# Megvii-CSG/MegReader

Hardware: AMD Instinct MI355X
Metric: training images/sec, CRNN-CTC 32x128 crops, batch 256 per GPU (higher is better)
Workload: dtype bf16; 1 GPU; CRNN + 1D-CTC training step (BASELINE.json configs[1]): 32x128 crops, T=33, C=38, Adam; global_batch=256, per_gpu_batch=256, parallelism=dp1, launch=hipGraph replay

## Files before the change

megreader_amd/csrc/stem.hip:

```cpp
#include "common.h"
#include "../../include/megreader_hip.h"

namespace mr {

constexpr int STEM_COUT = 64;
constexpr int STEM_BWD_GROUPS = 1024;

template <typename T> __device__ __forceinline__ float round_as(float v) { return to_f32(from_f32<T>(v)); }

template <typename T, int CIN>
__device__ __forceinline__ void stem_stage_patch(float* patch, const float* __restrict__ x, int n, int ph, int H,
                                                 int W) {
  const int PW = W + 2;
  for (int r = 0; r < 4; ++r) {
    const int row = 2 * ph - 1 + r;
    const bool rv = row >= 0 && row < H;
    for (int j = threadIdx.x; j < CIN * W; j += blockDim.x) {
      const int c = j / W, col = j - c * W;
      const float v = rv ? x[((long long)(n * CIN + c) * H + row) * W + col] : 0.f;
      patch[(r * PW + col + 1) * CIN + c] = round_as<T>(v);
    }
  }
  if (threadIdx.x < 4 * 2 * CIN) {
    const int r = threadIdx.x / (2 * CIN), rem = threadIdx.x - r * 2 * CIN;
    const int side = rem / CIN, c = rem - side * CIN;
    patch[(r * PW + (side ? W + 1 : 0)) * CIN + c] = 0.f;
  }
}

template <typename T, int CIN>
__global__ __launch_bounds__(256) void stem_fwd_kernel(const float* __restrict__ x, const float* __restrict__ w,
                                                       long long wsk, long long wsc, long long wsr, long long wss,
                                                       const float* __restrict__ bias, T* __restrict__ y,
                                                       unsigned char* __restrict__ code, int N, int H, int W) {
  extern __shared__ float patch[];
  constexpr int KT = 9 * CIN;
  const int lane = threadIdx.x & 63, wv = threadIdx.x >> 6, nwv = blockDim.x >> 6;
  const int Ho = H / 2, Wo = W / 2, PW = W + 2;
  float wr[KT];
#pragma unroll
  for (int dr = 0; dr < 3; ++dr)
#pragma unroll
    for (int ds = 0; ds < 3; ++ds)
#pragma unroll
      for (int c = 0; c < CIN; ++c)
        wr[(dr * 3 + ds) * CIN + c] = round_as<T>(w[lane * wsk + c * wsc + dr * wsr + ds * wss]);
  const float b = bias ? bias[lane] : 0.f;
  const int per = (Wo + nwv - 1) / nwv;
  for (int strip = blockIdx.x; strip < N * Ho; strip += gridDim.x) {
    const int n = strip / Ho, ph = strip - n * Ho;
    __syncthreads();
    stem_stage_patch<T, CIN>(patch, x, n, ph, H, W);
    __syncthreads();
    const int pw1 = min(Wo, (wv + 1) * per);
    for (int pw = wv * per; pw < pw1; ++pw) {
      float P[4][4 * CIN];
#pragma unroll
      for (int r = 0; r < 4; ++r)
#pragma unroll
        for (int i = 0; i < 4 * CIN; ++i) P[r][i] = patch[(r * PW + 2 * pw) * CIN + i];
      float best = 0.f;
      int q = 0;
#pragma unroll
      for (int qq = 0; qq < 4; ++qq) {
        const int a = qq >> 1, bq = qq & 1;
        float acc = b;
#pragma unroll
        for (int dr = 0; dr < 3; ++dr)
#pragma unroll
          for (int i = 0; i < 3 * CIN; ++i) acc = fmaf(wr[dr * 3 * CIN + i], P[a + dr][bq * CIN + i], acc);
        if (qq == 0 || acc > best) {
          best = acc;
          q = qq;
        }
      }
      const bool pos = best > 0.f;
      const long long o = ((long long)strip * Wo + pw) * STEM_COUT + lane;
      y[o] = from_f32<T>(pos ? best : 0.f);
      code[o] = (unsigned char)(q | (pos ? 4 : 0));
    }
  }
}

template <typename T, int CIN>
__global__ __launch_bounds__(256) void stem_bwd_kernel(const T* __restrict__ dy, const unsigned char* __restrict__ code,
                                                       const float* __restrict__ x, float* __restrict__ partial, int N,
                                                       int H, int W) {
  extern __shared__ float patch[];
  constexpr int KT = 9 * CIN;
  __shared__ float red[4][KT + 1][STEM_COUT];
  const int lane = threadIdx.x & 63, wv = threadIdx.x >> 6, nwv = blockDim.x >> 6;
  const int Ho = H / 2, Wo = W / 2, PW = W + 2;
  float acc[KT];
#pragma unroll
  for (int k = 0; k < KT; ++k) acc[k] = 0.f;
  float accb = 0.f;
  const int per = (Wo + nwv - 1) / nwv;
  for (int strip = blockIdx.x; strip < N * Ho; strip += gridDim.x) {
    const int n = strip / Ho, ph = strip - n * Ho;
    __syncthreads();
    stem_stage_patch<T, CIN>(patch, x, n, ph, H, W);
    __syncthreads();
    const int pw1 = min(Wo, (wv + 1) * per);
    for (int pw = wv * per; pw < pw1; ++pw) {
      const long long o = ((long long)strip * Wo + pw) * STEM_COUT + lane;
      const int cd = code[o];
      const float g = (cd & 4) ? to_f32(dy[o]) : 0.f;
      const int q = cd & 3;
      float P[4][4 * CIN];
#pragma unroll
      for (int r = 0; r < 4; ++r)
#pragma unroll
        for (int i = 0; i < 4 * CIN; ++i) P[r][i] = patch[(r * PW + 2 * pw) * CIN + i];
      accb += g;
#pragma unroll
      for (int qq = 0; qq < 4; ++qq) {
        const int a = qq >> 1, bq = qq & 1;
        const float gq = (q == qq) ? g : 0.f;
#pragma unroll
        for (int dr = 0; dr < 3; ++dr)
#pragma unroll
          for (int i = 0; i < 3 * CIN; ++i)
            acc[dr * 3 * CIN + i] = fmaf(gq, P[a + dr][bq * CIN + i], acc[dr * 3 * CIN + i]);
      }
    }
  }
  __syncthreads();
#pragma unroll
  for (int k = 0; k < KT; ++k) red[wv][k][lane] = acc[k];
  red[wv][KT][lane] = accb;
  __syncthreads();
  for (int i = threadIdx.x; i < (KT + 1) * STEM_COUT; i += blockDim.x) {
    const int k = i / STEM_COUT, o = i - k * STEM_COUT;
    float s = 0.f;
    for (int v = 0; v < nwv; ++v) s += red[v][k][o];
    partial[(long long)blockIdx.x * (KT + 1) * STEM_COUT + i] = s;
  }
}

template <int CIN>
__device__ __forceinline__ void stem_stage_patch_bf16(bf16_t* patch, const float* __restrict__ x, int n, int ph,
                                                      int H, int W) {
  const int PW = W + 2;
  const int wv = threadIdx.x >> 6, lane = threadIdx.x & 63;
  const int rbase = (wv & 1) * 2;
  for (int col = lane + 64 * (wv >> 1); col < W; col += 128) {
    float v[2][CIN];
#pragma unroll
    for (int rr = 0; rr < 2; ++rr) {
      const int row = 2 * ph - 1 + rbase + rr;
      const bool rv = row >= 0 && row < H;
#pragma unroll
      for (int c = 0; c < CIN; ++c) v[rr][c] = rv ? x[((long long)(n * CIN + c) * H + row) * W + col] : 0.f;
    }
#pragma unroll
    for (int rr = 0; rr < 2; ++rr)
#pragma unroll
      for (int c = 0; c < CIN; ++c) patch[((rbase + rr) * PW + col + 1) * CIN + c] = (bf16_t)v[rr][c];
  }
  if (threadIdx.x < 4 * 2 * CIN) {
    const int r = threadIdx.x / (2 * CIN), rem = threadIdx.x - r * 2 * CIN;
    const int side = rem / CIN, c = rem - side * CIN;
    patch[(r * PW + (side ? W + 1 : 0)) * CIN + c] = (bf16_t)0.f;
  }
}

template <int CIN>
__global__ void stem_pack_kernel(const float* __restrict__ w, long long wsk, long long wsc, long long wsr,
                                 long long wss, bf16_t* __restrict__ wpack) {
  constexpr int KT = 9 * CIN;
  for (int i = threadIdx.x; i < STEM_COUT * 32; i += blockDim.x) {
    const int ch = i >> 5, k = i & 31;
    const int dr = k / (3 * CIN), rem = k - dr * 3 * CIN, ds = rem / CIN, c = rem - ds * CIN;
    wpack[i] = (bf16_t)(k < KT ? w[ch * wsk + c * wsc + dr * wsr + ds * wss] : 0.f);
  }
}

template <int CIN>
__global__ __launch_bounds__(256, 3) void stem_fwd_mfma_kernel(const float* __restrict__ x,
                                                            const bf16_t* __restrict__ wpack,
                                                            const float* __restrict__ bias, bf16_t* __restrict__ y,
                                                            unsigned char* __restrict__ code, int N, int H, int W) {
  extern __shared__ float patch_raw[];
  bf16_t* patch = (bf16_t*)patch_raw;
  constexpr int KT = 9 * CIN;
  const int lane = threadIdx.x & 63, wv = threadIdx.x >> 6, l15 = lane & 15, lg = lane >> 4;
  const int Ho = H / 2, Wo = W / 2, PW = W + 2, ROW = PW * CIN;
  bf16x8 wf[4];
#pragma unroll
  for (int ct = 0; ct < 4; ++ct) {
    const int ch = (l15 >> 2) * 16 + ct * 4 + (l15 & 3);
    wf[ct] = *(const bf16x8*)(wpack + ch * 32 + 8 * lg);
  }
  f32x4 bv[4];
#pragma unroll
  for (int ct = 0; ct < 4; ++ct)
    bv[ct] = bias ? *(const f32x4*)(bias + lg * 16 + ct * 4) : f32x4{0.f, 0.f, 0.f, 0.f};
  int koff[8];
#pragma unroll
  for (int i = 0; i < 8; ++i) {
    const int k = 8 * lg + i;
    const int dr = k / (3 * CIN), rem = k - dr * 3 * CIN;
    koff[i] = k < KT ? dr * ROW + rem : 0;
  }

  for (int strip = blockIdx.x; strip < N * Ho; strip += gridDim.x) {
    const int n = strip / Ho, ph = strip - n * Ho;
    __syncthreads();
    stem_stage_patch_bf16<CIN>(patch, x, n, ph, H, W);
    __syncthreads();
    for (int pw0 = wv * 16; pw0 < Wo; pw0 += 64) {
      const int pw = pw0 + l15;
      bf16x8 xf[4];
#pragma unroll
      for (int qq = 0; qq < 4; ++qq) {
        const int base = ((qq >> 1) * PW + 2 * pw + (qq & 1)) * CIN;
#pragma unroll
        for (int i = 0; i < 8; ++i) xf[qq][i] = patch[base + koff[i]];
      }
      bf16_t yo[16];
      unsigned char co[16];
#pragma unroll
      for (int ct = 0; ct < 4; ++ct) {
        f32x4 acc[4];
#pragma unroll
        for (int qq = 0; qq < 4; ++qq)
          acc[qq] = __builtin_amdgcn_mfma_f32_16x16x32_bf16(wf[ct], xf[qq], f32x4{0.f, 0.f, 0.f, 0.f}, 0, 0, 0);
#pragma unroll
        for (int r = 0; r < 4; ++r) {
          const float a0 = acc[0][r], a1 = acc[1][r], a2 = acc[2][r], a3 = acc[3][r];
          const bool c1 = a1 > a0, c2 = a3 > a2;
          const float m01 = c1 ? a1 : a0, m23 = c2 ? a3 : a2;
          const bool c3 = m23 > m01;
          const int q = c3 ? (c2 ? 3 : 2) : (c1 ? 1 : 0);
          const float best = (c3 ? m23 : m01) + bv[ct][r];
          const bool pos = best > 0.f;
          yo[ct * 4 + r] = (bf16_t)(pos ? best : 0.f);
          co[ct * 4 + r] = (unsigned char)(pos ? (q | 4) : q);
        }
      }
      const long long o = ((long long)strip * Wo + pw) * STEM_COUT + lg * 16;
      *(uint4*)(y + o) = *(const uint4*)&yo[0];
      *(uint4*)(y + o + 8) = *(const uint4*)&yo[8];
      *(uint4*)(code + o) = *(const uint4*)&co[0];
    }
  }
}

template <int CIN>
__global__ __launch_bounds__(256, 4) void stem_bwd_mfma_kernel(const bf16_t* __restrict__ dy,
                                                            const unsigned char* __restrict__ code,
                                                            const float* __restrict__ x, float* __restrict__ partial,
                                                            int N, int H, int W) {
  extern __shared__ float patch_raw[];
  bf16_t* patch = (bf16_t*)patch_raw;
  const unsigned short* patch16 = (const unsigned short*)patch_raw;
  const unsigned short* dy16 = (const unsigned short*)dy;
  constexpr int KT = 9 * CIN;
  __shared__ float red[4][KT + 1][STEM_COUT];
  const int lane = threadIdx.x & 63, wv = threadIdx.x >> 6, l15 = lane & 15, lg = lane >> 4;
  const int Ho = H / 2, Wo = W / 2, PW = W + 2, ROW = PW * CIN;
  int xoff[2][8];
  unsigned xand[2], xor_[2];
#pragma unroll
  for (int nt = 0; nt < 2; ++nt) {
    const int k = l15 + 16 * nt;
    const int dr = k / (3 * CIN), rem = k - dr * 3 * CIN;
    xand[nt] = k < KT ? 0xFFFFFFFFu : 0u;
    xor_[nt] = k == KT ? 0x3F803F80u : 0u;
#pragma unroll
    for (int i = 0; i < 8; ++i) {
      const int px = 2 * lg + (i >> 2), qq = i & 3;
      xoff[nt][i] = k < KT ? ((qq >> 1) * PW + 2 * px + (qq & 1)) * CIN + dr * ROW + rem : 0;
    }
  }
  f32x4 acc[4][2];
#pragma unroll
  for (int mt = 0; mt < 4; ++mt)
#pragma unroll
    for (int nt = 0; nt < 2; ++nt) acc[mt][nt] = f32x4{0.f, 0.f, 0.f, 0.f};

  unsigned gd[4][2], gc[4][2];
  auto load_chunk = [&](int strip, int pw0) {
    const long long o = ((long long)strip * Wo + pw0 + 2 * lg) * STEM_COUT + l15;
#pragma unroll
    for (int mt = 0; mt < 4; ++mt)
#pragma unroll
      for (int h = 0; h < 2; ++h) {
        const long long oo = o + (long long)h * STEM_COUT + mt * 16;
        gd[mt][h] = dy16[oo];
        gc[mt][h] = code[oo];
      }
  };

  for (int strip = blockIdx.x; strip < N * Ho; strip += gridDim.x) {
    const int n = strip / Ho, ph = strip - n * Ho;
    if (wv * 8 < Wo) load_chunk(strip, wv * 8);
    __syncthreads();
    stem_stage_patch_bf16<CIN>(patch, x, n, ph, H, W);
    __syncthreads();
    for (int pw0 = wv * 8; pw0 < Wo; pw0 += 32) {
      u32x4 gf[4];
#pragma unroll
      for (int mt = 0; mt < 4; ++mt)
#pragma unroll
        for (int h = 0; h < 2; ++h) {
          const unsigned cd = gc[mt][h];
          const unsigned g = (cd & 4u) ? gd[mt][h] : 0u;
          const unsigned sh = g << ((cd & 1u) * 16u);
          gf[mt][h * 2 + 0] = (cd & 2u) ? 0u : sh;
          gf[mt][h * 2 + 1] = (cd & 2u) ? sh : 0u;
        }
      if (pw0 + 32 < Wo) load_chunk(strip, pw0 + 32);
      u32x4 xf[2];
#pragma unroll
      for (int nt = 0; nt < 2; ++nt)
#pragma unroll
        for (int d = 0; d < 4; ++d) {
          const unsigned lo = patch16[2 * pw0 * CIN + xoff[nt][2 * d]];
          const unsigned hi = patch16[2 * pw0 * CIN + xoff[nt][2 * d + 1]];
          xf[nt][d] = ((lo | (hi << 16)) & xand[nt]) | xor_[nt];
        }
#pragma unroll
      for (int mt = 0; mt < 4; ++mt)
#pragma unroll
        for (int nt = 0; nt < 2; ++nt)
          acc[mt][nt] = __builtin_amdgcn_mfma_f32_16x16x32_bf16(*(const bf16x8*)&gf[mt], *(const bf16x8*)&xf[nt],
                                                                acc[mt][nt], 0, 0, 0);
    }
  }
  __syncthreads();
#pragma unroll
  for (int mt = 0; mt < 4; ++mt)
#pragma unroll
    for (int nt = 0; nt < 2; ++nt) {
      const int k = l15 + 16 * nt;
      if (k <= KT)
#pragma unroll
        for (int r = 0; r < 4; ++r) red[wv][k][mt * 16 + lg * 4 + r] = acc[mt][nt][r];
    }
  __syncthreads();
  for (int i = threadIdx.x; i < (KT + 1) * STEM_COUT; i += blockDim.x) {
    const int k = i / STEM_COUT, oc = i - k * STEM_COUT;
    partial[(long long)blockIdx.x * (KT + 1) * STEM_COUT + i] = red[0][k][oc] + red[1][k][oc] + red[2][k][oc] + red[3][k][oc];
  }
}

template <int CIN>
__global__ __launch_bounds__(512) void stem_bwd_reduce_kernel(const float* __restrict__ partial, int G,
                                                              float* __restrict__ dw, long long dsk, long long dsc,
                                                              long long dsr, long long dss,
                                                              float* __restrict__ dbias) {
  constexpr int KT = 9 * CIN;
  __shared__ float red[8][STEM_COUT];
  const int k = blockIdx.x, o = threadIdx.x & 63, part = threadIdx.x >> 6;
  float s = 0.f;
  for (int g = blockIdx.y + 8 * part; g < G; g += 64) s += partial[((long long)g * (KT + 1) + k) * STEM_COUT + o];
  red[part][o] = s;
  __syncthreads();
  if (part == 0) {
#pragma unroll
    for (int p = 1; p < 8; ++p) s += red[p][o];
    if (k < KT) {
      const int c = k % CIN, t = k / CIN, ds = t % 3, dr = t / 3;
      if (dw) atomicAdd(&dw[o * dsk + c * dsc + dr * dsr + ds * dss], s);
    } else if (dbias) {
      atomicAdd(&dbias[o], s);
    }
  }
}

}

using namespace mr;

#define DISPATCH_T(dtype, ...)                                   \
  if ((dtype) == MR_F32) { typedef float T; __VA_ARGS__; }       \
  else if ((dtype) == MR_BF16) { typedef bf16_t T; __VA_ARGS__; } \
  else { mr::set_error("bad dtype %d", (dtype)); return MR_ERR_DTYPE; }

static int stem_check(const char* who, int N, int Cin, int H, int W) {
  if (!(N > 0 && (Cin == 1 || Cin == 3) && H >= 2 && W >= 2 && H % 2 == 0 && W % 2 == 0 &&
        4ll * (W + 2) * Cin * 4 <= 48 * 1024)) {
    mr::set_error("%s: unsupported shape N=%d Cin=%d H=%d W=%d (Cin in {1,3}, even H and W, W <= ~1000)", who, N,
                  Cin, H, W);
    return MR_ERR_ARG;
  }
  return MR_OK;
}

extern "C" {

long long mr_stem_bwd_workspace(int Cin) { return (long long)STEM_BWD_GROUPS * (9 * Cin + 1) * STEM_COUT; }

int mr_stem_pack(const float* w, long long wsk, long long wsc, long long wsr, long long wss, void* wpack, int Cin,
                 hipStream_t stream) {
  MR_CHECK_ARG(Cin == 1 || Cin == 3, "mr_stem_pack: Cin must be 1 or 3");
  if (Cin == 3)
    hipLaunchKernelGGL((stem_pack_kernel<3>), dim3(1), dim3(256), 0, stream, w, wsk, wsc, wsr, wss, (bf16_t*)wpack);
  else
    hipLaunchKernelGGL((stem_pack_kernel<1>), dim3(1), dim3(256), 0, stream, w, wsk, wsc, wsr, wss, (bf16_t*)wpack);
  MR_CHECK_LAUNCH();
  return MR_OK;
}

int mr_stem_fwd(int dtype, const float* x, const float* w, long long wsk, long long wsc, long long wsr,
                long long wss, const void* wpack, const float* bias, void* y, unsigned char* code, int N, int Cin,
                int H, int W, hipStream_t stream) {
  if (int rc = stem_check("mr_stem_fwd", N, Cin, H, W)) return rc;
  const size_t lds = sizeof(float) * 4 * (W + 2) * Cin;
  const int strips = N * (H / 2);
  const int grid = strips < 8192 ? strips : 8192;
  if (dtype == MR_BF16 && (W / 2) % 16 == 0 && wpack != nullptr) {
    if (Cin == 3)
      hipLaunchKernelGGL((stem_fwd_mfma_kernel<3>), dim3(grid), dim3(256), lds, stream, x, (const bf16_t*)wpack, bias,
                         (bf16_t*)y, code, N, H, W);
    else
      hipLaunchKernelGGL((stem_fwd_mfma_kernel<1>), dim3(grid), dim3(256), lds, stream, x, (const bf16_t*)wpack, bias,
                         (bf16_t*)y, code, N, H, W);
    MR_CHECK_LAUNCH();
    return MR_OK;
  }
  if (Cin == 3) {
    DISPATCH_T(dtype, hipLaunchKernelGGL((stem_fwd_kernel<T, 3>), dim3(grid), dim3(256), lds, stream, x, w, wsk, wsc,
                                         wsr, wss, bias, (T*)y, code, N, H, W));
  } else {
    DISPATCH_T(dtype, hipLaunchKernelGGL((stem_fwd_kernel<T, 1>), dim3(grid), dim3(256), lds, stream, x, w, wsk, wsc,
                                         wsr, wss, bias, (T*)y, code, N, H, W));
  }
  MR_CHECK_LAUNCH();
  return MR_OK;
}

int mr_stem_bwd(int dtype, const void* dy, const unsigned char* code, const float* x, float* workspace, float* dw,
                long long dsk, long long dsc, long long dsr, long long dss, float* dbias, int N, int Cin, int H,
                int W, hipStream_t stream) {
  if (int rc = stem_check("mr_stem_bwd", N, Cin, H, W)) return rc;
  MR_CHECK_ARG(workspace != nullptr, "mr_stem_bwd: workspace is null");
  const size_t lds = sizeof(float) * 4 * (W + 2) * Cin;
  const int strips = N * (H / 2);
  const int G = strips < STEM_BWD_GROUPS ? strips : STEM_BWD_GROUPS;
  if (dtype == MR_BF16 && (W / 2) % 16 == 0) {
    if (Cin == 3) {
      hipLaunchKernelGGL((stem_bwd_mfma_kernel<3>), dim3(G), dim3(256), lds, stream, (const bf16_t*)dy, code, x,
                         workspace, N, H, W);
      hipLaunchKernelGGL((stem_bwd_reduce_kernel<3>), dim3(9 * 3 + 1, 8), dim3(512), 0, stream, workspace, G, dw, dsk,
                         dsc, dsr, dss, dbias);
    } else {
      hipLaunchKernelGGL((stem_bwd_mfma_kernel<1>), dim3(G), dim3(256), lds, stream, (const bf16_t*)dy, code, x,
                         workspace, N, H, W);
      hipLaunchKernelGGL((stem_bwd_reduce_kernel<1>), dim3(9 * 1 + 1, 8), dim3(512), 0, stream, workspace, G, dw, dsk,
                         dsc, dsr, dss, dbias);
    }
    MR_CHECK_LAUNCH();
    return MR_OK;
  }
  if (Cin == 3) {
    DISPATCH_T(dtype, hipLaunchKernelGGL((stem_bwd_kernel<T, 3>), dim3(G), dim3(256), lds, stream, (const T*)dy, code,
                                         x, workspace, N, H, W));
    hipLaunchKernelGGL((stem_bwd_reduce_kernel<3>), dim3(9 * 3 + 1, 8), dim3(512), 0, stream, workspace, G, dw, dsk, dsc,
                       dsr, dss, dbias);
  } else {
    DISPATCH_T(dtype, hipLaunchKernelGGL((stem_bwd_kernel<T, 1>), dim3(G), dim3(256), lds, stream, (const T*)dy, code,
                                         x, workspace, N, H, W));
    hipLaunchKernelGGL((stem_bwd_reduce_kernel<1>), dim3(9 * 1 + 1, 8), dim3(512), 0, stream, workspace, G, dw, dsk, dsc,
                       dsr, dss, dbias);
  }
  MR_CHECK_LAUNCH();
  return MR_OK;
}

}
```

Before: 109,300 images/s.

## Stream stem conv rows through an LDS ring buffer with register prefetch

```diff
diff --git a/megreader_amd/csrc/stem.hip b/megreader_amd/csrc/stem.hip
--- a/megreader_amd/csrc/stem.hip
+++ b/megreader_amd/csrc/stem.hip
@@ -1,4 +1,5 @@
 #include "common.h"
+#include "device.h"
 #include "../../include/megreader_hip.h"
 
 namespace mr {
@@ -138,32 +139,60 @@
   }
 }
 
-template <int CIN>
-__device__ __forceinline__ void stem_stage_patch_bf16(bf16_t* patch, const float* __restrict__ x, int n, int ph,
-                                                      int H, int W) {
-  const int PW = W + 2;
-  const int wv = threadIdx.x >> 6, lane = threadIdx.x & 63;
-  const int rbase = (wv & 1) * 2;
-  for (int col = lane + 64 * (wv >> 1); col < W; col += 128) {
-    float v[2][CIN];
-#pragma unroll
-    for (int rr = 0; rr < 2; ++rr) {
-      const int row = 2 * ph - 1 + rbase + rr;
-      const bool rv = row >= 0 && row < H;
-#pragma unroll
-      for (int c = 0; c < CIN; ++c) v[rr][c] = rv ? x[((long long)(n * CIN + c) * H + row) * W + col] : 0.f;
-    }
-#pragma unroll
-    for (int rr = 0; rr < 2; ++rr)
-#pragma unroll
-      for (int c = 0; c < CIN; ++c) patch[((rbase + rr) * PW + col + 1) * CIN + c] = (bf16_t)v[rr][c];
-  }
-  if (threadIdx.x < 4 * 2 * CIN) {
-    const int r = threadIdx.x / (2 * CIN), rem = threadIdx.x - r * 2 * CIN;
-    const int side = rem / CIN, c = rem - side * CIN;
-    patch[(r * PW + (side ? W + 1 : 0)) * CIN + c] = (bf16_t)0.f;
-  }
-}
+constexpr int STEM_RING_SLOTS = 10;
+
+template <int CIN, int KPF>
+struct StemStager {
+  int plane[KPF];
+  int loff[KPF];
+  int rr[KPF];
+  int H, W, ROW;
+
+  __device__ __forceinline__ void init(int H_, int W_) {
+    H = H_, W = W_, ROW = (W + 2) * CIN;
+    const int W4 = W / 4, per_row = CIN * W4;
+#pragma unroll
+    for (int it = 0; it < KPF; ++it) {
+      const int j = it * 256 + threadIdx.x;
+      const int r = j / per_row, rem = j - r * per_row, c = rem / W4, col = 4 * (rem - c * W4);
+      rr[it] = r < 2 ? r : -1;
+      plane[it] = r < 2 ? c * H * W + col : 0;
+      loff[it] = r * ROW + (col + 1) * CIN + c;
+    }
+  }
+  __device__ __forceinline__ void load(const float* __restrict__ ximg, int t0, float4 (&v)[KPF], bool on = true) const {
+#pragma unroll
+    for (int it = 0; it < KPF; ++it) {
+      const int row = on ? min(max(t0 - 1 + rr[it], 0), H - 1) : 0;
+      v[it] = *(const float4*)(ximg + plane[it] + (long long)row * W);
+    }
+  }
+  __device__ __forceinline__ void store(bf16_t* ring, int t0, const float4 (&v)[KPF], bool on = true) const {
+    const int s0 = t0 & 7;
+#pragma unroll
+    for (int it = 0; it < KPF; ++it) {
+      float4 t = v[it];
+      asm volatile("" : "+v"(t.x), "+v"(t.y), "+v"(t.z), "+v"(t.w));
+      if (rr[it] < 0) continue;
+      const int row = t0 - 1 + rr[it];
+      if (!(on && row >= 0 && row < H)) t = float4{0.f, 0.f, 0.f, 0.f};
+      bf16_t* d = ring + s0 * ROW + loff[it];
+      const bf16_t b0 = (bf16_t)t.x, b1 = (bf16_t)t.y, b2 = (bf16_t)t.z, b3 = (bf16_t)t.w;
+      d[0] = b0, d[CIN] = b1, d[2 * CIN] = b2, d[3 * CIN] = b3;
+      if (s0 == 0) {
+        d += 8 * ROW;
+        d[0] = b0, d[CIN] = b1, d[2 * CIN] = b2, d[3 * CIN] = b3;
+      }
+    }
+  }
+  __device__ __forceinline__ void zero_pads(bf16_t* ring) const {
+    if (threadIdx.x < STEM_RING_SLOTS * 2 * CIN) {
+      const int s = threadIdx.x / (2 * CIN), rem = threadIdx.x - s * 2 * CIN;
+      const int side = rem / CIN, c = rem - side * CIN;
+      ring[(s * (W + 2) + (side ? W + 1 : 0)) * CIN + c] = (bf16_t)0.f;
+    }
+  }
+};
 
 template <int CIN>
 __global__ void stem_pack_kernel(const float* __restrict__ w, long long wsk, long long wsc, long long wsr,
@@ -176,15 +205,17 @@
   }
 }
 
-template <int CIN>
-__global__ __launch_bounds__(256, 3) void stem_fwd_mfma_kernel(const float* __restrict__ x,
+template <int CIN, int KPF>
+__global__ __launch_bounds__(256, KPF == 1 ? 3 : 2) void stem_fwd_mfma_kernel(const float* __restrict__ x,
                                                             const bf16_t* __restrict__ wpack,
                                                             const float* __restrict__ bias, bf16_t* __restrict__ y,
-                                                            unsigned char* __restrict__ code, int N, int H, int W) {
-  extern __shared__ float patch_raw[];
-  bf16_t* patch = (bf16_t*)patch_raw;
+                                                            unsigned char* __restrict__ code, int N, int H, int W,
+                                                            int R, int runs) {
+  extern __shared__ float ring_raw[];
+  bf16_t* ring = (bf16_t*)ring_raw;
   constexpr int KT = 9 * CIN;
-  const int lane = threadIdx.x & 63, wv = threadIdx.x >> 6, l15 = lane & 15, lg = lane >> 4;
+  const int lane = threadIdx.x & 63, l15 = lane & 15, lg = lane >> 4;
+  const int wv = __builtin_amdgcn_readfirstlane(threadIdx.x >> 6);
   const int Ho = H / 2, Wo = W / 2, PW = W + 2, ROW = PW * CIN;
   bf16x8 wf[4];
 #pragma unroll
@@ -203,62 +234,98 @@
     const int dr = k / (3 * CIN), rem = k - dr * 3 * CIN;
     koff[i] = k < KT ? dr * ROW + rem : 0;
   }
-
-  for (int strip = blockIdx.x; strip < N * Ho; strip += gridDim.x) {
-    const int n = strip / Ho, ph = strip - n * Ho;
-    __syncthreads();
-    stem_stage_patch_bf16<CIN>(patch, x, n, ph, H, W);
-    __syncthreads();
-    for (int pw0 = wv * 16; pw0 < Wo; pw0 += 64) {
-      const int pw = pw0 + l15;
-      bf16x8 xf[4];
-#pragma unroll
-      for (int qq = 0; qq < 4; ++qq) {
-        const int base = ((qq >> 1) * PW + 2 * pw + (qq & 1)) * CIN;
-#pragma unroll
-        for (int i = 0; i < 8; ++i) xf[qq][i] = patch[base + koff[i]];
-      }
-      bf16_t yo[16];
-      unsigned char co[16];
-#pragma unroll
-      for (int ct = 0; ct < 4; ++ct) {
-        f32x4 acc[4];
-#pragma unroll
-        for (int qq = 0; qq < 4; ++qq)
-          acc[qq] = __builtin_amdgcn_mfma_f32_16x16x32_bf16(wf[ct], xf[qq], f32x4{0.f, 0.f, 0.f, 0.f}, 0, 0, 0);
-#pragma unroll
-        for (int r = 0; r < 4; ++r) {
-          const float a0 = acc[0][r], a1 = acc[1][r], a2 = acc[2][r], a3 = acc[3][r];
-          const bool c1 = a1 > a0, c2 = a3 > a2;
-          const float m01 = c1 ? a1 : a0, m23 = c2 ? a3 : a2;
-          const bool c3 = m23 > m01;
-          const int q = c3 ? (c2 ? 3 : 2) : (c1 ? 1 : 0);
-          const float best = (c3 ? m23 : m01) + bv[ct][r];
-          const bool pos = best > 0.f;
-          yo[ct * 4 + r] = (bf16_t)(pos ? best : 0.f);
-          co[ct * 4 + r] = (unsigned char)(pos ? (q | 4) : q);
+  StemStager<CIN, KPF> st;
+  st.init(H, W);
+  st.zero_pads(ring);
+
+  const int units = N * runs;
+  for (int unit = blockIdx.x; unit < units; unit += gridDim.x) {
+    const int n = unit / runs, p0 = (unit - n * runs) * R, p1 = min(Ho, p0 + R);
+    const float* ximg = x + (long long)n * CIN * H * W;
+    float4 v[KPF];
+    {
+      float4 v2[KPF];
+      st.load(ximg, 2 * p0, v);
+      st.load(ximg, 2 * p0 + 2, v2);
+      st.store(ring, 2 * p0, v);
+      st.store(ring, 2 * p0 + 2, v2);
+    }
+    lds_barrier();
+    for (int p = p0; p < p1; ++p) {
+      const bool more = p + 1 < p1;
+      st.load(ximg, 2 * p + 4, v, more);
+      __builtin_amdgcn_sched_barrier(0);
+      const bf16_t* rows = ring + ((2 * p) & 7) * ROW;
+      const long long strip = (long long)n * Ho + p;
+      auto chunk = [&](int pw0, bool stage, bool live) __attribute__((always_inline)) {
+        const int pw = pw0 + l15;
+        bf16x8 xf[4];
+#pragma unroll
+        for (int qq = 0; qq < 4; ++qq) {
+          const int base = ((qq >> 1) * PW + 2 * pw + (qq & 1)) * CIN;
+#pragma unroll
+          for (int i = 0; i < 8; ++i) xf[qq][i] = rows[base + koff[i]];
         }
-      }
-      const long long o = ((long long)strip * Wo + pw) * STEM_COUT + lg * 16;
-      *(uint4*)(y + o) = *(const uint4*)&yo[0];
-      *(uint4*)(y + o + 8) = *(const uint4*)&yo[8];
-      *(uint4*)(code + o) = *(const uint4*)&co[0];
-    }
-  }
-}
-
-template <int CIN>
-__global__ __launch_bounds__(256, 4) void stem_bwd_mfma_kernel(const bf16_t* __restrict__ dy,
+        float yo[16];
+        unsigned co[16];
+#pragma unroll
+        for (int ct = 0; ct < 4; ++ct) {
+          f32x4 acc[4];
+#pragma unroll
+          for (int qq = 0; qq < 4; ++qq)
+            acc[qq] = __builtin_amdgcn_mfma_f32_16x16x32_bf16(wf[ct], xf[qq], f32x4{0.f, 0.f, 0.f, 0.f}, 0, 0, 0);
+#pragma unroll
+          for (int r = 0; r < 4; ++r) {
+            const float a0 = acc[0][r], a1 = acc[1][r], a2 = acc[2][r], a3 = acc[3][r];
+            const bool c1 = a1 > a0, c2 = a3 > a2;
+            const float m01 = c1 ? a1 : a0, m23 = c2 ? a3 : a2;
+            const bool c3 = m23 > m01;
+            const int q = c3 ? (c2 ? 3 : 2) : (c1 ? 1 : 0);
+            const float best = (c3 ? m23 : m01) + bv[ct][r];
+            const bool pos = best > 0.f;
+            yo[ct * 4 + r] = pos ? best : 0.f;
+            co[ct * 4 + r] = pos ? (q | 4) : q;
+          }
+        }
+        auto pk = [](float a, float b) { return __builtin_bit_cast(unsigned, bf16x2{(bf16_t)a, (bf16_t)b}); };
+        auto pc = [](const unsigned* c) { return c[0] | (c[1] << 8) | (c[2] << 16) | (c[3] << 24); };
+        const uint4 y0{pk(yo[0], yo[1]), pk(yo[2], yo[3]), pk(yo[4], yo[5]), pk(yo[6], yo[7])};
+        const uint4 y1{pk(yo[8], yo[9]), pk(yo[10], yo[11]), pk(yo[12], yo[13]), pk(yo[14], yo[15])};
+        const uint4 c0{pc(co), pc(co + 4), pc(co + 8), pc(co + 12)};
+        if (stage) {
+#pragma unroll
+          for (int it = 0; it < KPF; ++it)
+            asm volatile("" : "+v"(v[it].x), "+v"(v[it].y), "+v"(v[it].z), "+v"(v[it].w)
+                         : "v"(y0.x), "v"(y0.y), "v"(y0.z), "v"(y0.w), "v"(y1.x), "v"(y1.y), "v"(y1.z), "v"(y1.w),
+                           "v"(c0.x), "v"(c0.y), "v"(c0.z), "v"(c0.w));
+          st.store(ring, 2 * p + 4, v, more);
+        }
+        if (live) {
+          const long long o = (strip * Wo + pw) * STEM_COUT + lg * 16;
+          *(uint4*)(y + o) = y0;
+          *(uint4*)(y + o + 8) = y1;
+          *(uint4*)(code + o) = c0;
+        }
+      };
+      const bool live = wv * 16 < Wo;
+      chunk(live ? wv * 16 : 0, true, live);
+      for (int pw0 = wv * 16 + 64; pw0 < Wo; pw0 += 64) chunk(pw0, false, true);
+      lds_barrier();
+    }
+  }
+}
+
+template <int CIN, int KPF>
+__global__ __launch_bounds__(256, 2) void stem_bwd_mfma_kernel(const bf16_t* __restrict__ dy,
                                                             const unsigned char* __restrict__ code,
                                                             const float* __restrict__ x, float* __restrict__ partial,
-                                                            int N, int H, int W) {
-  extern __shared__ float patch_raw[];
-  bf16_t* patch = (bf16_t*)patch_raw;
-  const unsigned short* patch16 = (const unsigned short*)patch_raw;
-  const unsigned short* dy16 = (const unsigned short*)dy;
+                                                            int N, int H, int W, int R, int runs) {
+  extern __shared__ float ring_raw[];
+  bf16_t* ring = (bf16_t*)ring_raw;
   constexpr int KT = 9 * CIN;
   __shared__ float red[4][KT + 1][STEM_COUT];
-  const int lane = threadIdx.x & 63, wv = threadIdx.x >> 6, l15 = lane & 15, lg = lane >> 4;
+  const int lane = threadIdx.x & 63, l15 = lane & 15, lg = lane >> 4;
+  const int wv = __builtin_amdgcn_readfirstlane(threadIdx.x >> 6);
   const int Ho = H / 2, Wo = W / 2, PW = W + 2, ROW = PW * CIN;
   int xoff[2][8];
   unsigned xand[2], xor_[2];
@@ -279,57 +346,80 @@
   for (int mt = 0; mt < 4; ++mt)
 #pragma unroll
     for (int nt = 0; nt < 2; ++nt) acc[mt][nt] = f32x4{0.f, 0.f, 0.f, 0.f};
-
-  unsigned gd[4][2], gc[4][2];
-  auto load_chunk = [&](int strip, int pw0) {
-    const long long o = ((long long)strip * Wo + pw0 + 2 * lg) * STEM_COUT + l15;
-#pragma unroll
-    for (int mt = 0; mt < 4; ++mt)
-#pragma unroll
-      for (int h = 0; h < 2; ++h) {
-        const long long oo = o + (long long)h * STEM_COUT + mt * 16;
-        gd[mt][h] = dy16[oo];
-        gc[mt][h] = code[oo];
+  StemStager<CIN, KPF> st;
+  st.init(H, W);
+  st.zero_pads(ring);
+
+  uint2 gd[2];
+  unsigned gc[2];
+  auto load_chunk = [&](long long strip, int pw0) {
+    const long long o = (strip * Wo + pw0 + 2 * lg) * STEM_COUT + 4 * l15;
+#pragma unroll
+    for (int h = 0; h < 2; ++h) {
+      gd[h] = *(const uint2*)(dy + o + h * STEM_COUT);
+      gc[h] = *(const unsigned*)(code + o + h * STEM_COUT);
+    }
+  };
+
+  const int units = N * runs;
+  for (int unit = blockIdx.x; unit < units; unit += gridDim.x) {
+    const int n = unit / runs, p0 = (unit - n * runs) * R, p1 = min(Ho, p0 + R);
+    const float* ximg = x + (long long)n * CIN * H * W;
+    if (wv * 8 < Wo) load_chunk((long long)n * Ho + p0, wv * 8);
+    float4 v[KPF];
+    {
+      float4 v2[KPF];
+      st.load(ximg, 2 * p0, v);
+      st.load(ximg, 2 * p0 + 2, v2);
+      st.store(ring, 2 * p0, v);
+      st.store(ring, 2 * p0 + 2, v2);
+    }
+    lds_barrier();
+    for (int p = p0; p < p1; ++p) {
+      const bool more = p + 1 < p1;
+      st.load(ximg, 2 * p + 4, v, more);
+      __builtin_amdgcn_sched_barrier(0);
+      const unsigned short* rows = (const unsigned short*)ring + ((2 * p) & 7) * ROW;
+      const long long strip = (long long)n * Ho + p;
+      for (int pw0 = wv * 8; pw0 < Wo; pw0 += 32) {
+        u32x4 gf[4];
+#pragma unroll
+        for (int mt = 0; mt < 4; ++mt)
+#pragma unroll
+          for (int h = 0; h < 2; ++h) {
+            const unsigned pair = (mt & 2) ? gd[h].y : gd[h].x;
+            const unsigned cd = gc[h] >> (8 * mt);
+            const unsigned g = (cd & 4u) ? ((mt & 1) ? pair >> 16 : pair & 0xFFFFu) : 0u;
+            const unsigned sh = g << ((cd & 1u) * 16u);
+            gf[mt][h * 2 + 0] = (cd & 2u) ? 0u : sh;
+            gf[mt][h * 2 + 1] = (cd & 2u) ? sh : 0u;
+          }
+        if (pw0 + 32 < Wo) {
+          load_chunk(strip, pw0 + 32);
+        } else {
+          st.store(ring, 2 * p + 4, v, more);
+          if (more) load_chunk(strip + 1, wv * 8);
+        }
+        u32x4 xf[2];
+#pragma unroll
+        for (int nt = 0; nt < 2; ++nt)
+#pragma unroll
+          for (int d = 0; d < 4; ++d) {
+            const unsigned lo = rows[2 * pw0 * CIN + xoff[nt][2 * d]];
+            const unsigned hi = rows[2 * pw0 * CIN + xoff[nt][2 * d + 1]];
+            xf[nt][d] = ((lo | (hi << 16)) & xand[nt]) | xor_[nt];
+          }
+#pragma unroll
+        for (int mt = 0; mt < 4; ++mt)
+#pragma unroll
+          for (int nt = 0; nt < 2; ++nt)
+            acc[mt][nt] = __builtin_amdgcn_mfma_f32_16x16x32_bf16(*(const bf16x8*)&gf[mt], *(const bf16x8*)&xf[nt],
+                                                                  acc[mt][nt], 0, 0, 0);
       }
-  };
-
-  for (int strip = blockIdx.x; strip < N * Ho; strip += gridDim.x) {
-    const int n = strip / Ho, ph = strip - n * Ho;
-    if (wv * 8 < Wo) load_chunk(strip, wv * 8);
-    __syncthreads();
-    stem_stage_patch_bf16<CIN>(patch, x, n, ph, H, W);
-    __syncthreads();
-    for (int pw0 = wv * 8; pw0 < Wo; pw0 += 32) {
-      u32x4 gf[4];
-#pragma unroll
-      for (int mt = 0; mt < 4; ++mt)
-#pragma unroll
-        for (int h = 0; h < 2; ++h) {
-          const unsigned cd = gc[mt][h];
-          const unsigned g = (cd & 4u) ? gd[mt][h] : 0u;
-          const unsigned sh = g << ((cd & 1u) * 16u);
-          gf[mt][h * 2 + 0] = (cd & 2u) ? 0u : sh;
-          gf[mt][h * 2 + 1] = (cd & 2u) ? sh : 0u;
-        }
-      if (pw0 + 32 < Wo) load_chunk(strip, pw0 + 32);
-      u32x4 xf[2];
-#pragma unroll
-      for (int nt = 0; nt < 2; ++nt)
-#pragma unroll
-        for (int d = 0; d < 4; ++d) {
-          const unsigned lo = patch16[2 * pw0 * CIN + xoff[nt][2 * d]];
-          const unsigned hi = patch16[2 * pw0 * CIN + xoff[nt][2 * d + 1]];
-          xf[nt][d] = ((lo | (hi << 16)) & xand[nt]) | xor_[nt];
-        }
-#pragma unroll
-      for (int mt = 0; mt < 4; ++mt)
-#pragma unroll
-        for (int nt = 0; nt < 2; ++nt)
-          acc[mt][nt] = __builtin_amdgcn_mfma_f32_16x16x32_bf16(*(const bf16x8*)&gf[mt], *(const bf16x8*)&xf[nt],
-                                                                acc[mt][nt], 0, 0, 0);
-    }
-  }
-  __syncthreads();
+      if (wv * 8 >= Wo) st.store(ring, 2 * p + 4, v, more);
+      lds_barrier();
+    }
+  }
 #pragma unroll
   for (int mt = 0; mt < 4; ++mt)
 #pragma unroll
@@ -337,7 +427,7 @@
       const int k = l15 + 16 * nt;
       if (k <= KT)
 #pragma unroll
-        for (int r = 0; r < 4; ++r) red[wv][k][mt * 16 + lg * 4 + r] = acc[mt][nt][r];
+        for (int r = 0; r < 4; ++r) red[wv][k][4 * (lg * 4 + r) + mt] = acc[mt][nt][r];
     }
   __syncthreads();
   for (int i = threadIdx.x; i < (KT + 1) * STEM_COUT; i += blockDim.x) {
@@ -381,13 +471,78 @@
 
 static int stem_check(const char* who, int N, int Cin, int H, int W) {
   if (!(N > 0 && (Cin == 1 || Cin == 3) && H >= 2 && W >= 2 && H % 2 == 0 && W % 2 == 0 &&
-        4ll * (W + 2) * Cin * 4 <= 48 * 1024)) {
+        4ll * (W + 2) * Cin * 4 <= 48 * 1024 && (long long)Cin * H * W < (1ll << 31))) {
     mr::set_error("%s: unsupported shape N=%d Cin=%d H=%d W=%d (Cin in {1,3}, even H and W, W <= ~1000)", who, N,
                   Cin, H, W);
     return MR_ERR_ARG;
   }
   return MR_OK;
 }
+
+struct StemPlan { int R, runs, grid; };
+static StemPlan stem_plan(int N, int Ho, int slots) {
+  int runs = 1;
+  while (runs < Ho && (long long)N * runs < slots) ++runs;
+  StemPlan p;
+  p.R = (Ho + runs - 1) / runs;
+  p.runs = (Ho + p.R - 1) / p.R;
+  const long long units = (long long)N * p.runs;
+  p.grid = (int)(units < slots ? units : slots);
+  return p;
+}
+
+static size_t stem_ring_bytes(int Cin, int W) { return sizeof(bf16_t) * STEM_RING_SLOTS * (W + 2) * Cin; }
+
+template <typename K>
+static int stem_slots(const char* who, K kernel, size_t lds, int* slots) {
+  if (lds > 48 * 1024)
+    if (int rc = ensure_dynamic_lds(kernel, lds)) return rc;
+  int per_cu = 0;
+  if (hipOccupancyMaxActiveBlocksPerMultiprocessor(&per_cu, kernel, 256, lds) != hipSuccess || per_cu < 1) {
+    (void)hipGetLastError();
+    mr::set_error("%s: occupancy query failed", who);
+    return MR_ERR_LAUNCH;
+  }
+  *slots = num_cus() * per_cu;
+  return MR_OK;
+}
+
+template <int CIN, int KPF>
+static int stem_fwd_mfma(const float* x, const bf16_t* wpack, const float* bias, bf16_t* y, unsigned char* code, int N,
+                         int H, int W, hipStream_t stream) {
+  const size_t lds = stem_ring_bytes(CIN, W);
+  int slots = 0;
+  if (int rc = stem_slots("mr_stem_fwd", stem_fwd_mfma_kernel<CIN, KPF>, lds, &slots)) return rc;
+  const StemPlan p = stem_plan(N, H / 2, slots);
+  hipLaunchKernelGGL((stem_fwd_mfma_kernel<CIN, KPF>), dim3(p.grid), dim3(256), lds, stream, x, wpack, bias, y, code, N,
+                     H, W, p.R, p.runs);
+  MR_CHECK_LAUNCH();
+  return MR_OK;
+}
+
+template <int CIN, int KPF>
+static int stem_bwd_mfma(const bf16_t* dy, const unsigned char* code, const float* x, float* partial, int N, int H,
+                         int W, int* G, hipStream_t stream) {
+  const size_t lds = stem_ring_bytes(CIN, W);
+  int slots = 0;
+  if (int rc = stem_slots("mr_stem_bwd", stem_bwd_mfma_kernel<CIN, KPF>, lds, &slots)) return rc;
+  const StemPlan p = stem_plan(N, H / 2, slots < STEM_BWD_GROUPS ? slots : STEM_BWD_GROUPS);
+  hipLaunchKernelGGL((stem_bwd_mfma_kernel<CIN, KPF>), dim3(p.grid), dim3(256), lds, stream, dy, code, x, partial, N, H,
+                     W, p.R, p.runs);
+  MR_CHECK_LAUNCH();
+  *G = p.grid;
+  return MR_OK;
+}
+
+#define STEM_DISPATCH_KPF(CIN, W, ...)                                         \
+  {                                                                            \
+    const int items = 2 * (CIN) * ((W) / 4);                                   \
+    if (items <= 256) { constexpr int KPF = 1; __VA_ARGS__; }                  \
+    else if (items <= 512) { constexpr int KPF = 2; __VA_ARGS__; }             \
+    else { constexpr int KPF = 6; __VA_ARGS__; }                               \
+  }
+
+static bool aligned_to(const void* p, size_t a) { return ((size_t)p & (a - 1)) == 0; }
 
 extern "C" {
 
@@ -412,14 +567,16 @@
   const int strips = N * (H / 2);
   const int grid = strips < 8192 ? strips : 8192;
   if (dtype == MR_BF16 && (W / 2) % 16 == 0 && wpack != nullptr) {
-    if (Cin == 3)
-      hipLaunchKernelGGL((stem_fwd_mfma_kernel<3>), dim3(grid), dim3(256), lds, stream, x, (const bf16_t*)wpack, bias,
-                         (bf16_t*)y, code, N, H, W);
-    else
-      hipLaunchKernelGGL((stem_fwd_mfma_kernel<1>), dim3(grid), dim3(256), lds, stream, x, (const bf16_t*)wpack, bias,
-                         (bf16_t*)y, code, N, H, W);
-    MR_CHECK_LAUNCH();
-    return MR_OK;
+    MR_CHECK_ARG(aligned_to(x, 16) && aligned_to(wpack, 16) && aligned_to(y, 16) && aligned_to(code, 16) &&
+                     (bias == nullptr || aligned_to(bias, 16)),
+                 "mr_stem_fwd: the bf16 MFMA path needs 16-byte aligned x, wpack, bias, y and code");
+    int rc;
+    if (Cin == 3) {
+      STEM_DISPATCH_KPF(3, W, rc = (stem_fwd_mfma<3, KPF>(x, (const bf16_t*)wpack, bias, (bf16_t*)y, code, N, H, W, stream)));
+    } else {
+      STEM_DISPATCH_KPF(1, W, rc = (stem_fwd_mfma<1, KPF>(x, (const bf16_t*)wpack, bias, (bf16_t*)y, code, N, H, W, stream)));
+    }
+    return rc;
   }
   if (Cin == 3) {
     DISPATCH_T(dtype, hipLaunchKernelGGL((stem_fwd_kernel<T, 3>), dim3(grid), dim3(256), lds, stream, x, w, wsk, wsc,
@@ -441,15 +598,18 @@
   const int strips = N * (H / 2);
   const int G = strips < STEM_BWD_GROUPS ? strips : STEM_BWD_GROUPS;
   if (dtype == MR_BF16 && (W / 2) % 16 == 0) {
+    MR_CHECK_ARG(aligned_to(x, 16) && aligned_to(dy, 8) && aligned_to(code, 4),
+                 "mr_stem_bwd: the bf16 MFMA path needs 16-byte aligned x, 8-byte aligned dy and 4-byte aligned code");
+    int rc, Gm = 0;
     if (Cin == 3) {
-      hipLaunchKernelGGL((stem_bwd_mfma_kernel<3>), dim3(G), dim3(256), lds, stream, (const bf16_t*)dy, code, x,
-                         workspace, N, H, W);
-      hipLaunchKernelGGL((stem_bwd_reduce_kernel<3>), dim3(9 * 3 + 1, 8), dim3(512), 0, stream, workspace, G, dw, dsk,
+      STEM_DISPATCH_KPF(3, W, rc = (stem_bwd_mfma<3, KPF>((const bf16_t*)dy, code, x, workspace, N, H, W, &Gm, stream)));
+      if (rc) return rc;
+      hipLaunchKernelGGL((stem_bwd_reduce_kernel<3>), dim3(9 * 3 + 1, 8), dim3(512), 0, stream, workspace, Gm, dw, dsk,
                          dsc, dsr, dss, dbias);
     } else {
-      hipLaunchKernelGGL((stem_bwd_mfma_kernel<1>), dim3(G), dim3(256), lds, stream, (const bf16_t*)dy, code, x,
-                         workspace, N, H, W);
-      hipLaunchKernelGGL((stem_bwd_reduce_kernel<1>), dim3(9 * 1 + 1, 8), dim3(512), 0, stream, workspace, G, dw, dsk,
+      STEM_DISPATCH_KPF(1, W, rc = (stem_bwd_mfma<1, KPF>((const bf16_t*)dy, code, x, workspace, N, H, W, &Gm, stream)));
+      if (rc) return rc;
+      hipLaunchKernelGGL((stem_bwd_reduce_kernel<1>), dim3(9 * 1 + 1, 8), dim3(512), 0, stream, workspace, Gm, dw, dsk,
                          dsc, dsr, dss, dbias);
     }
     MR_CHECK_LAUNCH();
```

Measured after the change: 110,100 images/s (median of 6 runs). Within noise of the previous version (+0.8%).
